# OpenSim2Real/gym-os2r

Hardware: AMD Instinct MI355X
Metric: env-steps/sec (aggregate) monopod balance task (higher is better)
Workload: dtype f64; 1 GPU; C4: 65536 envs/GPU free_hip balancing, ground contact, per-env domain randomisation (C5 = 8 x C4); envs_per_gpu=65536, total_envs=65536, task_mode=free_hip, substeps=10, pgs_exact=12, preroll_steps=1000, contact=True, domain_randomisation=True, actions=U(-1,1) Philox on device, n_ranks_seen=1, splits=1, rollout_steps_per_launch=1

## Files before the change

gym-os2r_amd/csrc/os2r_capi.hip:

```cpp
#include <hip/hip_runtime.h>

#include <cfloat>
#include <cmath>
#include <cstdio>
#include <cstring>
#include <new>
#include <deque>
#include <mutex>
#include <string>
#include <vector>

#include "os2r_kernels.hpp"

using namespace os2r;

namespace os2r {
int static_model_id(const Os2rModel& m);
bool same_model(const Os2rModel& a, const Os2rModel& b);
}

struct JitEntry {
  Os2rModel model;
  int dtype = 0, device = 0;
  hipModule_t module = nullptr;
// ... 61 lines not shown
  int32_t* steps = nullptr;
  uint32_t* episode = nullptr;
  uint8_t* pose = nullptr;
  void* solver_l = nullptr;
  uint32_t* solver_flags = nullptr;
  unsigned int* violations = nullptr;
  void *b_obs = nullptr, *b_rew = nullptr, *b_term = nullptr;
  unsigned long long* counters = nullptr;
  uint8_t* b_done = nullptr;
  hipEvent_t ev0 = nullptr, ev1 = nullptr;
  uint16_t* reason = nullptr;
  uint8_t* done_mask = nullptr;
  uint32_t* mirror_host = nullptr;
  uint32_t* mirror_dev = nullptr;
  unsigned long long* debug = nullptr;
  void* pol_act = nullptr;
  uint8_t* pol_open = nullptr;
  void* copy_stage = nullptr;
};

}

struct Os2rSim : SimBase {};

namespace {

#define HIP_TRY(sim, expr)                                                                     \
  do {                                                                                         \
    hipError_t _e = (expr);                                                                    \
    if (_e != hipSuccess) {                                                                    \
      (sim)->err = std::string(#expr) + ": " + hipGetErrorString(_e);                          \
      return OS2R_ERR_HIP;                                                                     \
    }                                                                                          \
  } while (0)

template <typename T>
void fill_model(const Os2rModel& m_in, bool contact, DevModel<T>& d) {
  Os2rModel m = m_in;
  if (!contact) m.ncand = 0;
  std::memset(&d, 0, sizeof(d));
  d.nq = m.nq;
  for (int i = 0; i < OS2R_MAX_DOF; ++i) {
    d.axis[i] = m.axis[i];
    for (int k = 0; k < 9; ++k) d.rfix[i][k] = (T)m.rfix[i][k];
    for (int k = 0; k < 3; ++k) { d.rpos[i][k] = (T)m.rpos[i][k]; d.com[i][k] = (T)m.com[i][k]; }
    for (int k = 0; k < 6; ++k) d.icom[i][k] = (T)m.icom[i][k];
    d.mass[i] = (T)m.mass[i];
    d.damping[i] = (T)m.damping[i];
    d.friction[i] = (T)m.friction[i];
    d.mu[i] = (T)m.mu[i];
  }
  for (int k = 0; k < 2; ++k) { d.act_dof[k] = m.act_dof[k]; d.max_torque[k] = (T)m.max_torque[k]; }
  d.gravity_z = (T)m.gravity_z;
  int k = 0;
  for (int b = 0; b < OS2R_MAX_DOF; ++b) {
    d.cand_begin[b] = k;
    while (k < m.ncand && m.cand_body[k] == b) ++k;
  }
  d.cand_begin[OS2R_MAX_DOF] = k;
  for (int c = 0; c < m.ncand; ++c)
    for (int j = 0; j < 3; ++j) d.cand_p[c][j] = (T)m.cand_p[c][j];
  for (int b = 0; b < OS2R_MAX_DOF; ++b) {
    for (int j = 0; j < 3; ++j) d.cand_center[b][j] = (T)m.cand_center[b][j];
    d.cand_radius[b] = m.cand_radius[b] > 0.0 ? (T)(m.cand_radius[b] * 1.000001) : (T)1e30;
  }
}

inline float float_at_or_above(double v) {
  float f = (float)v;
  if ((double)f < v) f = std::nextafter(f, FLT_MAX);
  return f;
}
inline float float_at_or_below(double v) {
  float f = (float)v;
  if ((double)f > v) f = std::nextafter(f, -FLT_MAX);
  return f;
}
inline void done_bounds(int kind, double lo, double hi, double& dlo, double& dhi) { dlo = lo; dhi = hi; }
inline void done_bounds(int kind, double lo, double hi, float& dlo, float& dhi) {
  const bool periodic = kind == OS2R_OBS_POS_PERIODIC_NORM || kind == OS2R_OBS_POS_PERIODIC_RAW;
  dlo = periodic ? float_at_or_below(lo) : float_at_or_above(lo);
  dhi = periodic ? float_at_or_above(hi) : float_at_or_below(hi);
}

template <typename T>
void fill_task(const Os2rConfig& cfg, DevTask<T>& d) {
  const Os2rTaskSpec& t = cfg.task;
  std::memset(&d, 0, sizeof(d));
  d.obs_dim = t.obs_dim;
  for (int i = 0; i < OS2R_MAX_OBS; ++i) {
    d.obs_kind[i] = t.obs_kind[i];
    d.obs_src[i] = t.obs_src[i];
    d.obs_low[i] = (T)t.obs_low[i];
    d.obs_high[i] = (T)t.obs_high[i];
    done_bounds(t.obs_kind[i], t.done_lo[i], t.done_hi[i], d.done_lo[i], d.done_hi[i]);
  }
  d.reward_id = t.reward_id; d.normalized = t.normalized;
  d.idx_pitch_pos = t.idx_pitch_pos; d.idx_yaw_vel = t.idx_yaw_vel;
  d.idx_hip_pos = t.idx_hip_pos; d.idx_knee_pos = t.idx_knee_pos;
  d.max_episode_steps = t.max_episode_steps;
  d.reset_mode = t.reset_mode; d.n_reset_poses = t.n_reset_poses;
  for (int i = 0; i < OS2R_MAX_RESET_POSES; ++i) {
    d.reset_pose_id[i] = t.reset_pose_id[i]; d.reset_laying[i] = t.reset_laying[i];
    d.reset_pitch[i] = t.reset_pitch[i]; d.reset_hip[i] = t.reset_hip[i]; d.reset_knee[i] = t.reset_knee[i];
  }
  d.reset_simple = t.reset_simple;
  for (int i = 0; i < 6; ++i) d.leg_def[i] = t.leg_def[i];
  d.dof_yaw = t.dof_yaw; d.dof_pitch = t.dof_pitch; d.dof_bc = t.dof_bc; d.dof_hip = t.dof_hip; d.dof_knee = t.dof_knee;
  d.randomize_params = t.randomize_params;
  d.gravity_rollouts = t.gravity_rollouts;
  d.dr_gravity_mean = t.dr_gravity_mean; d.dr_gravity_std = t.dr_gravity_std;
  d.dr_mass_lo = t.dr_mass_lo; d.dr_mass_hi = t.dr_mass_hi;
  d.dr_friction_lo = t.dr_friction_lo; d.dr_friction_hi = t.dr_friction_hi;
  d.dr_damping_lo = t.dr_damping_lo; d.dr_damping_hi = t.dr_damping_hi;
// ... 784 lines not shown
```

gym-os2r_amd/csrc/os2r_device.hpp:

```cpp
#pragma once
#include <type_traits>
#include <hip/hip_runtime.h>
#include <stdint.h>

#include "../../include/os2r.h"
#include "os2r_models_gen.hpp"

namespace os2r {

constexpr int kWave = 64;
template <typename T> struct StdSolver { static constexpr int kNormalIters = 2; static constexpr bool kExact = true; };
template <> struct StdSolver<float> { static constexpr int kNormalIters = 2; static constexpr bool kExact = false; };
__host__ __device__ constexpr int warm_first(int) { return 3; }
__host__ __device__ constexpr int sweep_cap_base(int nq) { return nq >= 5 ? 6 : 4; }
constexpr int kExactRounds = 8;
constexpr unsigned kCarryJoints = 0x80000000u;
template <typename T, int NQ_> struct SolverCarry {
  unsigned act = 0u;
  T ln[NQ_] = {}, lx[NQ_] = {}, ly[NQ_] = {}, lf[NQ_] = {};
};
template <typename T> __host__ __device__ constexpr int std_iters(int nq) { return sizeof(T) == 8 ? sweep_cap_base(nq) + kExactRounds : 20; }
template <typename T> __host__ __device__ inline bool is_std_solver(int iters, int normal_iters, int exact, int nq) {
  return iters == std_iters<T>(nq) && normal_iters == StdSolver<T>::kNormalIters && (exact > 0) == StdSolver<T>::kExact;
}
constexpr int kPgsGroup = 4;
constexpr int kExactProx = 2;
constexpr double kExactEps = 1e-6, kExactSnap = 1e-12;
constexpr double kExactIncons = 1e-4, kExactNoBound = 1e300;

struct WorkCounts {
  unsigned scanned = 0;
  unsigned row_bodies = 0;
  unsigned body_sweeps = 0;
  unsigned sweeps = 0;
  unsigned lane_contacts = 0;
  unsigned live_lane_sweeps = 0;
  unsigned full_sincos = 0;
  unsigned exact_solves = 0;
  unsigned lane_exact_solves = 0;
};

template <typename T>
struct DevModel {
  int nq;
  int axis[OS2R_MAX_DOF];
  T rfix[OS2R_MAX_DOF][9];
  T rpos[OS2R_MAX_DOF][3];
  T mass[OS2R_MAX_DOF];
  T com[OS2R_MAX_DOF][3];
  T icom[OS2R_MAX_DOF][6];
  T damping[OS2R_MAX_DOF];
  T friction[OS2R_MAX_DOF];
  T mu[OS2R_MAX_DOF];
  int act_dof[2];
  T max_torque[2];
  T gravity_z;
  int cand_begin[OS2R_MAX_DOF + 1];
  T cand_p[OS2R_MAX_CAND][3];
  T cand_center[OS2R_MAX_DOF][3];
  T cand_radius[OS2R_MAX_DOF];
};

template <typename T>
struct DevTask {
  int obs_dim;
  int obs_kind[OS2R_MAX_OBS];
  int obs_src[OS2R_MAX_OBS];
  T obs_low[OS2R_MAX_OBS];
  T obs_high[OS2R_MAX_OBS];
  T done_lo[OS2R_MAX_OBS];
  T done_hi[OS2R_MAX_OBS];
  int reward_id, normalized;
  int idx_pitch_pos, idx_yaw_vel, idx_hip_pos, idx_knee_pos;
  int max_episode_steps;
  int reset_mode, n_reset_poses;
  int reset_pose_id[OS2R_MAX_RESET_POSES];
  int reset_laying[OS2R_MAX_RESET_POSES];
  double reset_pitch[OS2R_MAX_RESET_POSES];
  double reset_hip[OS2R_MAX_RESET_POSES];
  double reset_knee[OS2R_MAX_RESET_POSES];
  int reset_simple;
  double leg_def[6];
  int dof_yaw, dof_pitch, dof_bc, dof_hip, dof_knee;
  int randomize_params;
  int gravity_rollouts;
  double dr_gravity_mean, dr_gravity_std;
  double dr_mass_lo, dr_mass_hi, dr_friction_lo, dr_friction_hi, dr_damping_lo, dr_damping_hi;
  double dr_mu_base, dr_mu_lo, dr_mu_hi;
  double nominal_damping[OS2R_MAX_DOF];
};

#define OS2R_CONST __attribute__((address_space(4)))
template <typename T> using ModelPtr = const OS2R_CONST DevModel<T>*;
template <typename T> using TaskPtr = const OS2R_CONST DevTask<T>*;
template <typename T> __device__ __forceinline__ ModelPtr<T> as_const(const DevModel<T>* p) { return (ModelPtr<T>)p; }
template <typename T> __device__ __forceinline__ TaskPtr<T> as_const(const DevTask<T>* p) { return (TaskPtr<T>)p; }

template <typename T>
struct StepArgs {
  const DevModel<T>* __restrict__ model;
  const DevTask<T>* __restrict__ task;
  long long N;
  long long env_offset;
  unsigned long long seed;
  unsigned long long step_count;
  int substeps;
  int rollout_steps;
  int pgs_iters;
  int pgs_normal_iters;
  int pgs_exact;
  int auto_reset;
  T dt, erp, max_erv, margin, gravity_z;
  T pgs_tol;
// ... 2 lines not shown
  T* __restrict__ hist;
  T* __restrict__ mass_scale;
  T* __restrict__ damping;
  T* __restrict__ friction;
  T* __restrict__ mu;
  T* __restrict__ gravity;
  int32_t* __restrict__ steps;
  uint32_t* __restrict__ episode;
  uint8_t* __restrict__ pose;
  T* __restrict__ solver_l;
  uint32_t* __restrict__ solver_flags;
  unsigned int* __restrict__ violations;
  const T* __restrict__ actions;
  T* __restrict__ obs;
  T* __restrict__ reward;
  uint8_t* __restrict__ done;
  T* __restrict__ term_obs;
  const uint8_t* __restrict__ reset_mask;
  unsigned long long* __restrict__ debug;
  unsigned long long* __restrict__ counters;
  uint16_t* __restrict__ reason;
  uint8_t* __restrict__ done_mask;
  uint32_t* __restrict__ mirror;
  unsigned long long layout_kinds, layout_srcs;
  int layout_dim;
};

template <typename T, int NQ_>
struct RtModel {
  static constexpr int NQ = NQ_;
  static constexpr unsigned CMASK = (1u << NQ_) - 1u;
  static constexpr bool kStatic = false;
  ModelPtr<T> p;
  __device__ __forceinline__ int axis(int i) const { return p->axis[i]; }
  __device__ __forceinline__ T rfix(int i, int k) const { return p->rfix[i][k]; }
  __device__ __forceinline__ T rpos(int i, int k) const { return p->rpos[i][k]; }
  __device__ __forceinline__ T mass(int i) const { return p->mass[i]; }
  __device__ __forceinline__ T com(int i, int k) const { return p->com[i][k]; }
  __device__ __forceinline__ T icom(int i, int k) const { return p->icom[i][k]; }
  __device__ __forceinline__ T damping(int i) const { return p->damping[i]; }
  __device__ __forceinline__ T friction(int i) const { return p->friction[i]; }
  __device__ __forceinline__ T mu(int i) const { return p->mu[i]; }
  __device__ __forceinline__ int act_dof(int k) const { return p->act_dof[k]; }
  __device__ __forceinline__ T max_torque(int k) const { return p->max_torque[k]; }
  __device__ __forceinline__ int cand_begin(int b) const { return p->cand_begin[b]; }
  __device__ __forceinline__ T cand(int k, int j) const { return p->cand_p[k][j]; }
  __device__ __forceinline__ T cand_center(int b, int j) const { return p->cand_center[b][j]; }
  __device__ __forceinline__ T cand_radius(int b) const { return p->cand_radius[b]; }
};

template <int ID>
struct CandMeta {
  using Tb = gen::Tables<ID>;
  struct Data { int axis[OS2R_MAX_DOF]; bool starts[OS2R_MAX_CAND > 0 ? OS2R_MAX_CAND : 1]; };
  static constexpr int runs(int b, int a) {
    int n = 0;
    for (int k = Tb::cand_begin[b]; k < Tb::cand_begin[b + 1]; ++k)
      if (k == Tb::cand_begin[b] || Tb::cand_p[k][a] != Tb::cand_p[k - 1][a]) ++n;
    return n;
  }
  static constexpr Data make() {
    Data d{};
    for (int b = 0; b < Tb::nq; ++b) {
      int best = 0;
      for (int a = 1; a < 3; ++a)
        if (runs(b, a) < runs(b, best)) best = a;
      d.axis[b] = best;
      for (int k = Tb::cand_begin[b]; k < Tb::cand_begin[b + 1]; ++k)
        d.starts[k] = k == Tb::cand_begin[b] || Tb::cand_p[k][best] != Tb::cand_p[k - 1][best];
    }
    return d;
  }
  static constexpr Data value = make();
};

template <typename T, int ID>
struct StModel {
  using Tb = gen::Tables<ID>;
  static constexpr int NQ = Tb::nq;
  static constexpr unsigned CMASK = Tb::cmask;
  static constexpr bool kStatic = true;
  __device__ __forceinline__ constexpr int axis(int i) const { return Tb::axis[i]; }
  __device__ __forceinline__ constexpr T rfix(int i, int k) const { return (T)Tb::rfix[i][k]; }
  __device__ __forceinline__ constexpr T rpos(int i, int k) const { return (T)Tb::rpos[i][k]; }
  __device__ __forceinline__ constexpr T mass(int i) const { return (T)Tb::mass[i]; }
  __device__ __forceinline__ constexpr T com(int i, int k) const { return (T)Tb::com[i][k]; }
  __device__ __forceinline__ constexpr T icom(int i, int k) const { return (T)Tb::icom[i][k]; }
  __device__ __forceinline__ constexpr T damping(int i) const { return (T)Tb::damping[i]; }
  __device__ __forceinline__ constexpr T friction(int i) const { return (T)Tb::friction[i]; }
  __device__ __forceinline__ constexpr T mu(int i) const { return (T)Tb::mu[i]; }
  __device__ __forceinline__ constexpr int act_dof(int k) const { return Tb::act_dof[k]; }
  __device__ __forceinline__ constexpr T max_torque(int k) const { return (T)Tb::max_torque[k]; }
  __device__ __forceinline__ constexpr int cand_begin(int b) const { return Tb::cand_begin[b]; }
  __device__ __forceinline__ constexpr T cand(int k, int j) const { return (T)Tb::cand_p[k][j]; }
  __device__ __forceinline__ constexpr T cand_center(int b, int j) const { return (T)Tb::cand_center[b][j]; }
  __device__ __forceinline__ constexpr T cand_radius(int b) const { return (T)Tb::cand_radius[b]; }
  static constexpr int cand_group_axis(int b) { return CandMeta<ID>::value.axis[b]; }
  static constexpr bool cand_starts_run(int , int k, int ) { return CandMeta<ID>::value.starts[k]; }
};

enum { kStreamAction = 1, kStreamReset = 2, kStreamParams = 3, kStreamGravity = 4, kStreamPolicyNoise = 5 };

__device__ __forceinline__ void philox4x32_10(uint32_t c0, uint32_t c1, uint32_t c2, uint32_t c3,
                                               uint32_t k0, uint32_t k1, uint32_t (&out)[4]) {
#pragma unroll
  for (int r = 0; r < 10; ++r) {
    const uint32_t hi0 = __umulhi(0xD2511F53u, c0), lo0 = 0xD2511F53u * c0;
    const uint32_t hi1 = __umulhi(0xCD9E8D57u, c2), lo1 = 0xCD9E8D57u * c2;
    const uint32_t n0 = hi1 ^ c1 ^ k0, n2 = hi0 ^ c3 ^ k1;
    c0 = n0; c1 = lo1; c2 = n2; c3 = lo0;
    k0 += 0x9E3779B9u; k1 += 0xBB67AE85u;
  }
  out[0] = c0; out[1] = c1; out[2] = c2; out[3] = c3;
}

__device__ __forceinline__ double u53(uint32_t a, uint32_t b) {
  return ((double)(a >> 5) * 67108864.0 + (double)(b >> 6)) / 9007199254740992.0;
}

__device__ __forceinline__ void uniform2(unsigned long long seed, uint32_t env, uint32_t stream,
                                          uint32_t ctr, uint32_t blk, double& u0, double& u1) {
  uint32_t o[4];
  philox4x32_10(env, stream, ctr, blk, (uint32_t)(seed & 0xffffffffull), (uint32_t)(seed >> 32), o);
  u0 = u53(o[0], o[1]);
  u1 = u53(o[2], o[3]);
}

__device__ __forceinline__ void normal2(unsigned long long seed, uint32_t env, uint32_t stream,
                                         uint32_t ctr, uint32_t blk, double& z0, double& z1) {
  double u0, u1;
  uniform2(seed, env, stream, ctr, blk, u0, u1);
  const double r = sqrt(-2.0 * log(1.0 - u0));
  const double th = 6.283185307179586476925286766559 * u1;
  z0 = r * cos(th);
  z1 = r * sin(th);
}

template <typename T>
struct V3 {
  T x, y, z;
};
template <typename T> __device__ __forceinline__ V3<T> mk(T x, T y, T z) { return V3<T>{x, y, z}; }
template <typename T> __device__ __forceinline__ V3<T> operator+(V3<T> a, V3<T> b) { return {a.x + b.x, a.y + b.y, a.z + b.z}; }
template <typename T> __device__ __forceinline__ V3<T> operator-(V3<T> a, V3<T> b) { return {a.x - b.x, a.y - b.y, a.z - b.z}; }
template <typename T> __device__ __forceinline__ V3<T> operator*(T s, V3<T> a) { return {s * a.x, s * a.y, s * a.z}; }
template <typename T> __device__ __forceinline__ T dot(V3<T> a, V3<T> b) { return a.x * b.x + a.y * b.y + a.z * b.z; }
template <typename T> __device__ __forceinline__ V3<T> cross(V3<T> a, V3<T> b) {
  return {a.y * b.z - a.z * b.y, a.z * b.x - a.x * b.z, a.x * b.y - a.y * b.x};
}
template <typename T> __device__ __forceinline__ T comp(V3<T> a, int k) { return k == 0 ? a.x : (k == 1 ? a.y : a.z); }
template <typename T> __device__ __forceinline__ void add_comp(V3<T>& a, int k, T v) {
// ... 153 lines not shown
  __device__ __forceinline__ T damping(int i) const { return slots[(1 * NQ + i) * kWave]; }
  __device__ __forceinline__ T friction(int i) const { return slots[(2 * NQ + i) * kWave]; }
  __device__ __forceinline__ T mu(int i) const { return slots[(3 * NQ + i) * kWave]; }
  __device__ __forceinline__ T gravity() const { return g; }
};

constexpr int kStamps = 32;
#if defined(OS2R_STAMPS) && defined(OS2R_STAMPS_LIGHT)
#define OS2R_STAMP(idx) do { } while (0)
#elif defined(OS2R_STAMPS)
#define OS2R_STAMP(idx)                                                                        \
  do {                                                                                         \
    __builtin_amdgcn_sched_barrier(0);                                                         \
    unsigned long long t_;                                                                     \
    asm volatile("s_memtime %0\n\ts_waitcnt lgkmcnt(0)" : "=s"(t_)::"memory");                 \
    __builtin_amdgcn_sched_barrier(0);                                                         \
    stamps[idx] += t_ - stamp_prev;                                                            \
    stamp_prev = t_;                                                                           \
  } while (0)
#elif defined(OS2R_PHASE_MARKS)
#define OS2R_STAMP(idx) asm volatile("s_nop 15\n\ts_nop %0\n\ts_nop %1" :: "i"((idx) % 8), "i"((idx) / 8) : "memory")
#else
#define OS2R_STAMP(idx) do { } while (0)
#endif

#ifdef OS2R_ISA_MARKS
#define OS2R_ISA_MARK(n) asm volatile("s_nop " #n ::: "memory")
#else
#define OS2R_ISA_MARK(n) do { } while (0)
#endif

constexpr int kPinVmem = 0x1 | 0x2 | 0x4 | 0x8 | 0x80 | 0x100 | 0x200 | 0x400;

constexpr int kPinDs = 0x1 | 0x2 | 0x4 | 0x8 | 0x10 | 0x20 | 0x40 | 0x400;

__device__ __forceinline__ double opaque(double x) { asm volatile("" : "+v"(x)); return x; }
__device__ __forceinline__ float opaque(float x) { asm volatile("" : "+v"(x)); return x; }

template <typename T> __device__ __forceinline__ T pick3(int k, T a, T b, T c) { return k == 0 ? a : (k == 1 ? b : c); }

template <typename T, typename MD>
__device__ __forceinline__ void joint_rotation(const MD& md, int i, T s_, T c_, T (&R)[9]) {
  const T s = opaque(s_), c = opaque(c_);
  const int ax = md.axis(i);
  const int ca = ax == 0 ? 1 : (ax == 1 ? 2 : 0);
  const int cb = ax == 0 ? 2 : (ax == 1 ? 0 : 1);
#pragma unroll
  for (int r = 0; r < 3; ++r) {
    const T fa = md.rfix(i, 3 * r + ca), fb = md.rfix(i, 3 * r + cb);
    const T keep = md.rfix(i, 3 * r + ax), va = c * fa + s * fb, vb = c * fb - s * fa;
#pragma unroll
    for (int j = 0; j < 3; ++j) R[3 * r + j] = j == ax ? keep : (j == ca ? va : vb);
  }
}

template <unsigned CMASK, int NB>
__device__ __forceinline__ constexpr int next_cand_body(int b) {
  for (int k = b + 1; k < NB; ++k)
    if ((CMASK >> k) & 1u) return k;
  return NB;
}
template <int B, int NB, unsigned CMASK, typename F>
__device__ __forceinline__ bool for_body(int b, F&& f) {
  if constexpr (B < NB) {
    if constexpr (((CMASK >> B) & 1u) && __builtin_popcount(CMASK >> B) <= 3) {
      if (b == B) { f(std::integral_constant<int, B>{}); return true; }
    }
    return for_body<B + 1, NB, CMASK>(b, f);
  } else {
    return false;
  }
}

enum { kSolverBoth = 0, kSolverExact = 1, kSolverSweeps = 2 };
template <typename T, typename MD, bool CONTACT, bool DR, bool COUNT = false, int SOLVER = kSolverBoth>
__device__ __forceinline__ void substep(const MD& md, const Params<T, MD, DR>& par,
                                        T (&q)[MD::NQ], T (&qd)[MD::NQ], T (&sn)[MD::NQ], T (&cs)[MD::NQ], bool first_iteration,
                                        T tau_hip, T tau_knee, T dt, T erp,
                                        T max_erv, T margin, int pgs_iters, int pgs_normal_iters, int pgs_exact, T pgs_tol, T* __restrict__ lds,
                                        const T* __restrict__ cand_lds, ModelPtr<T> mconst, WorkCounts& wc, SolverCarry<T, MD::NQ>& carry
#ifdef OS2R_STAMPS
                                        , unsigned long long (&stamps)[kStamps], unsigned long long& stamp_prev
#endif
                                        ) {
  constexpr int NQ = MD::NQ;
  constexpr unsigned CMASK = CONTACT ? MD::CMASK : 0u;
  const T inv_dt = rcp_t(dt);
  const T m_first = par.mass(NQ - 1), damp_first = par.damping(NQ - 1);
  __builtin_amdgcn_sched_barrier(DR ? kPinDs : kPinVmem);
  {
    bool ok = true, small = !first_iteration;
#pragma unroll
    for (int i = 0; i < NQ; ++i) { ok = ok && sincos_in_range(q[i]); small = small && fabs_t(dt * qd[i]) < T(0.06); }
    if constexpr (COUNT) wc.full_sincos += __ballot(!small) != 0ull ? 1u : 0u;
    if (small) {
#pragma unroll
      for (int i = 0; i < NQ; ++i) {
        const T d = dt * qd[i], z = d * d;
        T p = fma_t(z, T(-1.0 / 39916800.0), T(1.0 / 362880.0));
        p = fma_t(z, p, T(-1.0 / 5040.0));
        p = fma_t(z, p, T(1.0 / 120.0));
        p = fma_t(z, p, T(-1.0 / 6.0));
        const T sd = fma_t(d * z, p, d);
        T r = fma_t(z, T(-1.0 / 3628800.0), T(1.0 / 40320.0));
        r = fma_t(z, r, T(-1.0 / 720.0));
        r = fma_t(z, r, T(1.0 / 24.0));
// ... 234 lines not shown
#pragma unroll
      for (int r = i; r < NQ; ++r) Lc[r][i] = r == i ? sdi : uk[r][i] * sdi;
    }
  }
  OS2R_STAMP(19);

  OS2R_STAMP(2);
  T fb[NQ];
  T mub[NB];
#pragma unroll
  for (int j = 0; j < NQ; ++j) fb[j] = par.friction(j);
#pragma unroll
  for (int b = 0; b < NB; ++b) mub[b] = ((CMASK >> b) & 1u) ? par.mu(b) : T(0);
  __builtin_amdgcn_sched_barrier(DR ? kPinDs : kPinVmem);
  T y[NQ];
  T idj[NQ];
#pragma unroll
  for (int j = 0; j < NQ; ++j) {
    T mjj = 0;
#pragma unroll
    for (int k = 0; k <= j; ++k) { mjj += Lc[j][k] * Lc[j][k]; Lcs(j, k) = Lc[j][k]; }
    idj[j] = mjj > T(0) ? rcp_t(mjj) : T(0);
  }
#pragma unroll
  for (int i = 0; i < NQ; ++i) {
    T acc_ = vs[i];
#pragma unroll
    for (int k = 0; k < i; ++k) acc_ -= Lc[i][k] * y[k];
    y[i] = opaque(acc_ * Ldi[i]);
  }
  constexpr bool kStdExact = sizeof(T) == 8 && SOLVER == kSolverExact && MD::kStatic;
  constexpr bool kParkY0 = sizeof(T) == 8 && !kStdExact && (SOLVER != kSolverSweeps || !MD::kStatic);
  constexpr int kY0Slot = NQ * (NQ + 1) / 2 + 3 * NQ + NQ;
  static_assert(kY0Slot + NQ <= 8 * NQ, "per-lane LDS slots");
  T y0[NQ];
#pragma unroll
  for (int i = 0; i < NQ; ++i) {
    if constexpr (kParkY0) L(kY0Slot + i) = y[i];
    else y0[i] = y[i];
  }

  OS2R_STAMP(3);
  T dn[NB], dx[NB], dy[NB], erv[NB];
  T Gr[NB][3][NQ];
  bool act[NB];
  bool wave_act[NB];
#pragma unroll
  for (int b = 0; b < NB; ++b) { act[b] = false; wave_act[b] = false; }
  if (CMASK != 0u) {
    T Rw[9], ow[3];
    V3<T> aw[NQ], jo[NQ];
#pragma unroll
    for (int b = 0; b < NB; ++b) {
      constexpr int CHS = 4;
      T bA[3 * CHS], bB[3 * CHS];
      auto request = [&](int kk, int kend, T (&d)[3 * CHS]) {
#pragma unroll
        for (int j = 0; j < 3 * CHS; ++j) d[j] = (kk + j / 3 < kend) ? mconst->cand_p[kk + j / 3][j % 3] : T(0);
      };
      if constexpr (MD::kStatic) {
        if ((CMASK >> b) & 1u) {
          request(md.cand_begin(b), md.cand_begin(b + 1), bA);
          asm volatile("" ::: "memory");
        }
      }
      const V3<T> r = mk(md.rpos(b, 0), md.rpos(b, 1), md.rpos(b, 2));
      T Rb[9];
      joint_rotation<T>(md, b, sn[b], cs[b], Rb);
      if (b == 0) {
#pragma unroll
        for (int k = 0; k < 9; ++k) Rw[k] = Rb[k];
        ow[0] = r.x; ow[1] = r.y; ow[2] = r.z;
      } else {
        const V3<T> t = rmul(Rw, r);
        ow[0] += t.x; ow[1] += t.y; ow[2] += t.z;
        T n[9];
#pragma unroll
        for (int i = 0; i < 3; ++i)
#pragma unroll
          for (int j = 0; j < 3; ++j) n[3 * i + j] = Rw[3 * i] * Rb[j] + Rw[3 * i + 1] * Rb[3 + j] + Rw[3 * i + 2] * Rb[6 + j];
#pragma unroll
        for (int k = 0; k < 9; ++k) Rw[k] = n[k];
      }
      const int ax = md.axis(b);
      aw[b] = mk(pick3(ax, Rw[0], Rw[1], Rw[2]), pick3(ax, Rw[3], Rw[4], Rw[5]), pick3(ax, Rw[6], Rw[7], Rw[8]));
      jo[b] = mk(ow[0], ow[1], ow[2]);
      if (!((CMASK >> b) & 1u)) continue;
      OS2R_STAMP(4);
      const int k0 = md.cand_begin(b), k1 = md.cand_begin(b + 1);
      T W = 0, sx = 0, sy = 0, sz = 0;
      const T zc = Rw[6] * md.cand_center(b, 0) + Rw[7] * md.cand_center(b, 1) + Rw[8] * md.cand_center(b, 2) + ow[2];
      const bool near = zc - md.cand_radius(b) < margin;
      if constexpr (MD::kStatic) {
#pragma unroll
        for (int j = 0; j < 3 * CHS; ++j) asm volatile("" : "+s"(bA[j]));
        asm volatile("" ::: "memory");
      }
      if constexpr (COUNT) wc.scanned += __ballot(near) != 0ull ? 1u : 0u;
      if (__ballot(near) != 0ull)
      {
        constexpr int CH = 4;
        auto fetch = [&](int k, T (&d)[3 * CH]) {
#pragma unroll
          for (int j = 0; j < 3 * CH; ++j) d[j] = cand_lds[3 * k + j];
        };
        auto consume = [&](const T (&d)[3 * CH]) {
#pragma unroll
          for (int c = 0; c < CH; ++c) {
            const T px = d[3 * c], py = d[3 * c + 1], pz = d[3 * c + 2];
            const T z = Rw[6] * px + Rw[7] * py + Rw[8] * pz + ow[2];
            const T wgt = fmax_t(margin - z, T(0));
            W += wgt; sx += wgt * px; sy += wgt * py; sz += wgt * pz;
          }
        };
        if constexpr (MD::kStatic) {
          const T mo = margin - ow[2];
          auto arrived = [&](T (&d)[3 * CH]) {
#pragma unroll
            for (int j = 0; j < 3 * CH; ++j) asm volatile("" : "+s"(d[j]));
            asm volatile("" ::: "memory");
          };
          const int ga = MD::cand_group_axis(b), a1 = (ga + 1) % 3, a2 = (ga + 2) % 3;
          T S[3] = {T(0), T(0), T(0)};
          T Wg = T(0), pg = T(0), base = mo;
          auto weigh = [&](const T (&d)[3 * CH], int kk) {
#pragma unroll
            for (int c = 0; c < CH; ++c) {
              if (kk + c < k1) {
                if (MD::cand_starts_run(b, kk + c, ga)) {
                  W += Wg; S[ga] = fma_t(pg, Wg, S[ga]);
                  Wg = T(0); pg = d[3 * c + ga];
                  base = fma_t(-Rw[6 + ga], pg, mo);
                }
                const T p1 = d[3 * c + a1], p2 = d[3 * c + a2];
                const T mz = fma_t(-Rw[6 + a1], p1, fma_t(-Rw[6 + a2], p2, base));
                const T wgt = fmax_t(mz, T(0));
                Wg += wgt; S[a1] = fma_t(wgt, p1, S[a1]); S[a2] = fma_t(wgt, p2, S[a2]);
              }
            }
          };
          static_assert(CH == CHS, "chunk size of the request issued ahead");
#pragma unroll
          for (int kk = k0; kk < k1; kk += 2 * CH) {
            arrived(bA);
            if (kk + CH < k1) request(kk + CH, k1, bB);
            weigh(bA, kk);
            if (kk + CH < k1) {
              arrived(bB);
              if (kk + 2 * CH < k1) request(kk + 2 * CH, k1, bA);
              weigh(bB, kk + CH);
            }
          }
          W += Wg; S[ga] = fma_t(pg, Wg, S[ga]);
          sx = S[0]; sy = S[1]; sz = S[2];
        } else {
        T bufA[3 * CH], bufB[3 * CH];
        int k = k0;
        const int kpair = k0 + ((k1 - k0) / (2 * CH)) * (2 * CH);
        if (k < kpair) {
          fetch(k, bufA);
#pragma unroll 1
          for (; k < kpair; k += 2 * CH) {
            fetch(k + CH, bufB);
            consume(bufA);
            if (k + 2 * CH < kpair) fetch(k + 2 * CH, bufA);
            consume(bufB);
          }
        }
#pragma unroll 1
        for (; k < k1; ++k) {
          const T px = cand_lds[3 * k], py = cand_lds[3 * k + 1], pz = cand_lds[3 * k + 2];
          const T z = Rw[6] * px + Rw[7] * py + Rw[8] * pz + ow[2];
          const T wgt = fmax_t(margin - z, T(0));
          W += wgt; sx += wgt * px; sy += wgt * py; sz += wgt * pz;
        }
        }
      }
      OS2R_STAMP(5);
      act[b] = W > T(0);
      wave_act[b] = __ballot(act[b]) != 0ull;
      if constexpr (COUNT) { wc.row_bodies += wave_act[b] ? 1u : 0u; wc.lane_contacts += (unsigned)__popcll(__ballot(act[b])); }
      if (wave_act[b]) {
        T lcb[NQ][NQ];
#pragma unroll
        for (int j = 0; j < NQ; ++j)
#pragma unroll
          for (int k = 0; k < NQ; ++k)
            if (j <= b && k <= j) lcb[j][k] = Lcs(j, k);
        __builtin_amdgcn_sched_barrier(kPinDs);
        const T iw = act[b] ? rcp_t(W) : T(0);
        const V3<T> pc = mk(sx * iw, sy * iw, sz * iw);
        const V3<T> pw = rmul(Rw, pc) + jo[b];
        const T gap = pw.z;
        const T e = erp * (-gap) * inv_dt;
        erv[b] = gap >= T(0) ? -gap * inv_dt : (e > max_erv ? max_erv : e);
        T Jn[NQ], Jx[NQ], Jy[NQ];
#pragma unroll
        for (int j = 0; j < NQ; ++j) {
          if (j <= b) {
            const V3<T> c = cross(aw[j], pw - jo[j]);
            Jx[j] = c.x; Jy[j] = c.y; Jn[j] = c.z;
          }
        }
// ... 492 lines not shown
```

gym-os2r_amd/csrc/os2r_pybind.cpp:

```cpp
#include <pybind11/pybind11.h>
#include <pybind11/stl.h>

#include <cstdint>

#include "../../include/os2r.h"

namespace py = pybind11;
using addr = std::uintptr_t;

static Os2rSim* H(addr h) { return reinterpret_cast<Os2rSim*>(h); }
static void* P(addr a) { return reinterpret_cast<void*>(a); }

PYBIND11_MODULE(_os2r_py, m) {
  m.doc() = "pybind11 binding of libos2r.so (MI355X batched monopod stepper)";
  const auto nogil = py::call_guard<py::gil_scoped_release>();
  m.def("abi_version", &os2r_abi_version);
  m.def("abi_minor", &os2r_abi_minor);
  m.def("create", [](addr cfg) {
    Os2rSim* s = nullptr;
    int rc;
    { py::gil_scoped_release rel; rc = os2r_create(reinterpret_cast<const Os2rConfig*>(cfg), &s); }
    return py::make_tuple(rc, reinterpret_cast<addr>(s));
  });
  m.def("destroy", [](addr h) { return os2r_destroy(H(h)); }, nogil);
  m.def("reset", [](addr h, addr mask, addr obs, addr st) { return os2r_reset(H(h), (const uint8_t*)P(mask), P(obs), P(st)); }, nogil);
  m.def("step", [](addr h, addr act, addr obs, addr rew, addr done, addr term, addr st) {
    return os2r_step(H(h), P(act), P(obs), P(rew), (uint8_t*)P(done), P(term), P(st)); }, nogil);
  m.def("rollout", [](addr h, int n, addr act, addr obs, addr rew, addr done, addr term, addr why, addr st) {
    return os2r_rollout(H(h), n, P(act), P(obs), P(rew), (uint8_t*)P(done), P(term), (uint16_t*)P(why), P(st)); }, nogil);
  m.def("rollout_policy", [](addr h, int n, addr w, int flags, addr ret, addr len, addr obs, addr rew, addr done, addr term, addr why,
                             addr st) {
    return os2r_rollout_policy(H(h), n, P(w), flags, P(ret), (int32_t*)P(len), P(obs), P(rew), (uint8_t*)P(done), P(term),
                               (uint16_t*)P(why), P(st)); }, nogil);
  m.def("rollout_policy_noisy", [](addr h, int n, addr w, int flags, addr sigma, uint32_t salt, addr ret, addr len, addr obs, addr rew,
                                   addr done, addr term, addr why, addr act, addr eps, addr st) {
    return os2r_rollout_policy_noisy(H(h), n, P(w), flags, P(sigma), salt, P(ret), (int32_t*)P(len), P(obs), P(rew), (uint8_t*)P(done),
                                     P(term), (uint16_t*)P(why), P(act), P(eps), P(st)); }, nogil);
  m.def("rollout_policy_scheduled", [](addr h, int n, addr w, int period, int first, int flags, addr sigma, uint32_t salt, addr ret,
                                       addr len, addr obs, addr rew, addr done, addr term, addr why, addr act, addr eps, addr st) {
    return os2r_rollout_policy_scheduled(H(h), n, P(w), period, first, flags, P(sigma), salt, P(ret), (int32_t*)P(len), P(obs), P(rew),
                                         (uint8_t*)P(done), P(term), (uint16_t*)P(why), P(act), P(eps), P(st)); }, nogil);
  m.def("copy_envs", [](addr dst, addr src, addr index, int what, addr obs, addr st) {
    return os2r_copy_envs(H(dst), H(src), (const int32_t*)P(index), what, P(obs), P(st)); }, nogil);
  m.def("linearize", [](addr h, addr act, double eq, double ev, double ea, addr next, addr ja, addr jb, addr st) {
    const double eps[3] = {eq, ev, ea};
    return os2r_linearize(H(h), P(act), eps, P(next), P(ja), P(jb), P(st)); }, nogil);
  m.def("get_solver_state", [](addr h, addr l, addr f, addr st) { return os2r_get_solver_state(H(h), P(l), (uint32_t*)P(f), P(st)); }, nogil);
  m.def("set_solver_state", [](addr h, addr l, addr f, addr st) { return os2r_set_solver_state(H(h), P(l), (const uint32_t*)P(f), P(st)); }, nogil);
  m.def("get_state", [](addr h, addr q, addr qd, addr st) { return os2r_get_state(H(h), P(q), P(qd), P(st)); }, nogil);
  m.def("set_state", [](addr h, addr q, addr qd, addr st) { return os2r_set_state(H(h), P(q), P(qd), P(st)); }, nogil);
  m.def("get_action_history", [](addr h, int w, addr o, addr st) { return os2r_get_action_history(H(h), w, P(o), P(st)); }, nogil);
  m.def("set_action_history", [](addr h, int w, addr i, addr st) { return os2r_set_action_history(H(h), w, P(i), P(st)); }, nogil);
  m.def("set_params", [](addr h, int f, addr s, addr st) { return os2r_set_params(H(h), f, P(s), P(st)); }, nogil);
  m.def("get_params", [](addr h, int f, addr d, addr st) { return os2r_get_params(H(h), f, P(d), P(st)); }, nogil);
  m.def("get_episode_info", [](addr h, addr s, addr e, addr p, addr st) {
    return os2r_get_episode_info(H(h), (int32_t*)P(s), (uint32_t*)P(e), (uint8_t*)P(p), P(st)); }, nogil);
  m.def("set_episode_info", [](addr h, addr s, addr e, addr p, addr st) {
    return os2r_set_episode_info(H(h), (const int32_t*)P(s), (const uint32_t*)P(e), (const uint8_t*)P(p), P(st)); }, nogil);
  m.def("get_action_violations", [](addr h, addr d, int clear, addr st) {
    return os2r_get_action_violations(H(h), (uint32_t*)P(d), clear, P(st)); }, nogil);
  m.def("get_step_count", [](addr h) { uint64_t v = 0; int rc = os2r_get_step_count(H(h), &v); return py::make_tuple(rc, v); });
  m.def("set_step_count", [](addr h, uint64_t v) { return os2r_set_step_count(H(h), v); });
  m.def("bench_steps", [](addr h, int n, addr st) {
    float ms = 0.f;
    int rc;
    { py::gil_scoped_release rel; rc = os2r_bench_steps(H(h), n, P(st), &ms); }
    return py::make_tuple(rc, ms);
  });
  m.def("bench_enqueue", [](addr h, int n, addr st) {
    py::gil_scoped_release rel;
    return os2r_bench_steps(H(h), n, P(st), nullptr);
  });
  m.def("bench_steps_multi", [](std::vector<addr> hs, std::vector<addr> sts, int n) {
    std::vector<Os2rSim*> sims; std::vector<void*> streams;
    for (addr h : hs) sims.push_back(H(h));
    for (addr s : sts) streams.push_back(P(s));
    if (sims.size() != streams.size()) return (int)OS2R_ERR_INVALID;
    py::gil_scoped_release rel;
    return os2r_bench_steps_multi(sims.data(), streams.data(), (int)sims.size(), n);
  });
  m.def("set_work_counters", [](addr h, addr buf) { return os2r_set_work_counters(H(h), (uint64_t*)P(buf)); });
  m.def("set_done_reasons", [](addr h, addr buf) { return os2r_set_done_reasons(H(h), (uint16_t*)P(buf)); });
  m.def("set_done_mask", [](addr h, addr buf) { return os2r_set_done_mask(H(h), (uint8_t*)P(buf)); });
  m.def("get_violation_mirror", [](addr h) { const volatile uint32_t* w = nullptr; int rc = os2r_get_violation_mirror(H(h), &w); return py::make_tuple(rc, (addr)w); });
  m.def("model_is_compiled_in", [](addr model) { return os2r_model_is_compiled_in((const Os2rModel*)P(model)); });
  m.def("register_model_kernels", [](addr model, int dtype, int device, const std::string& path) {
    return os2r_register_model_kernels((const Os2rModel*)P(model), dtype, device, path.c_str()); });
  m.def("last_error", [](addr h) { return std::string(os2r_last_error(H(h))); });
}
```

gym-os2r_amd/jit.py:

```python
from __future__ import annotations

import ctypes as C
import hashlib
import os
import shutil
import subprocess
import tempfile
import warnings

from . import abi

_HERE = os.path.dirname(os.path.abspath(__file__))
CSRC = os.path.join(_HERE, "csrc")
ARCH = "gfx950"
FLAGS = ["-O3", "-std=c++17", "-fno-signed-zeros", "-fno-honor-nans", "-fno-honor-infinities", "-fno-slp-vectorize",
         "-mllvm", "-disable-machine-licm", "-mllvm", "-disable-machine-sink"]
_registered = set()


def enabled() -> bool:
    return os.environ.get("OS2R_JIT", "1") not in ("0", "false", "off", "")


def hipcc_path():
# ... 11 lines not shown

def _hx(x) -> str:
    return float(x).hex()


def table_source(m: abi.Os2rModel, table_id: int = 100) -> str:
    nq, nc = int(m.nq), int(m.ncand)
    begins, k = [], 0
    for b in range(nq):
        begins.append(k)
        while k < nc and m.cand_body[k] == b:
            k += 1
    begins.append(k)
    if k != nc:
        raise ValueError("candidate points must be grouped by body in ascending order")
    cmask = 0
    for c in range(nc):
        cmask |= 1 << int(m.cand_body[c])

    def arr1(vals):
        return "{" + ", ".join(vals) + "}"

    def arr2(rows):
        return "{" + ", ".join(arr1([_hx(v) for v in r]) for r in rows) + "}"

    cand = [[m.cand_p[c][j] for j in range(3)] for c in range(nc)] or [[0.0, 0.0, 0.0]]
    out = ["// GENERATED by gym_os2r_amd/jit.py -- the constants of one robot, numbers only.", "#pragma once",
           "namespace os2r { namespace gen {", f"template <> struct Tables<{table_id}> {{",
           f"  static constexpr int nq = {nq};",
           f"  static constexpr unsigned cmask = {cmask}u;",
           f"  static constexpr int axis[{nq}] = {arr1([str(int(m.axis[i])) for i in range(nq)])};",
           f"  static constexpr double rfix[{nq}][9] = {arr2([[m.rfix[i][k] for k in range(9)] for i in range(nq)])};",
           f"  static constexpr double rpos[{nq}][3] = {arr2([[m.rpos[i][k] for k in range(3)] for i in range(nq)])};",
           f"  static constexpr double mass[{nq}] = {arr1([_hx(m.mass[i]) for i in range(nq)])};",
           f"  static constexpr double com[{nq}][3] = {arr2([[m.com[i][k] for k in range(3)] for i in range(nq)])};",
           f"  static constexpr double icom[{nq}][6] = {arr2([[m.icom[i][k] for k in range(6)] for i in range(nq)])};",
           f"  static constexpr double damping[{nq}] = {arr1([_hx(m.damping[i]) for i in range(nq)])};",
           f"  static constexpr double friction[{nq}] = {arr1([_hx(m.friction[i]) for i in range(nq)])};",
           f"  static constexpr double mu[{nq}] = {arr1([_hx(m.mu[i]) for i in range(nq)])};",
           f"  static constexpr int act_dof[2] = {{{int(m.act_dof[0])}, {int(m.act_dof[1])}}};",
           f"  static constexpr double max_torque[2] = {{{_hx(m.max_torque[0])}, {_hx(m.max_torque[1])}}};",
           f"  static constexpr int ncand = {nc};",
           f"  static constexpr int cand_begin[{nq + 1}] = {arr1([str(v) for v in begins])};",
           f"  static constexpr double cand_p[{max(nc, 1)}][3] = {arr2(cand)};",
           f"  static constexpr double cand_center[{nq}][3] = "
           f"{arr2([[m.cand_center[i][k] for k in range(3)] for i in range(nq)])};",
           f"  static constexpr double cand_radius[{nq}] = {arr1([_hx(m.cand_radius[i]) for i in range(nq)])};",
           "};", "} }  // namespace os2r::gen", ""]
    return "\n".join(out)


def _sources_digest() -> str:
    h = hashlib.sha256()
    for name in ("os2r_device.hpp", "os2r_kernels.hpp", "os2r_models_gen.hpp", "os2r_jit_unit.hip"):
        with open(os.path.join(CSRC, name), "rb") as f:
            h.update(f.read())
    with open(os.path.join(os.path.dirname(_HERE), "include", "os2r.h"), "rb") as f:
        h.update(f.read())
    return h.hexdigest()


def task_layout(task: abi.Os2rTaskSpec):
    dim = int(task.obs_dim)
    if not 0 < dim <= abi.MAX_OBS or any(not 0 <= int(task.obs_kind[d]) < 16 or not 0 <= int(task.obs_src[d]) < 16 for d in range(dim)):
        return None
    kinds = sum(int(task.obs_kind[d]) << (4 * d) for d in range(dim))
    srcs = sum(int(task.obs_src[d]) << (4 * d) for d in range(dim))
    return kinds, srcs, dim


def code_object_path(m: abi.Os2rModel, dtype: int, contact: bool, layout=None) -> str:
    h = hashlib.sha256()
    h.update(table_source(m).encode())
    h.update(f"{dtype}|{int(bool(contact))}|{layout if contact else None}|{ARCH}|{' '.join(FLAGS)}|{_sources_digest()}".encode())
    return os.path.join(cache_dir(), f"os2r_{h.hexdigest()[:24]}.hsaco")


def build(m: abi.Os2rModel, dtype: int, contact: bool, force: bool = False, layout=None) -> str:
    out = code_object_path(m, dtype, contact, layout)
    if os.path.exists(out) and not force:
        return out
    hipcc = hipcc_path()
    if hipcc is None:
        raise RuntimeError("hipcc not found (set HIPCC or install ROCm): cannot specialise the kernels")
    real = "double" if dtype == abi.F64 else "float"
    with tempfile.TemporaryDirectory(prefix="os2r_jit_") as tmp:
        tab = os.path.join(tmp, "os2r_jit_tables.hpp")
        with open(tab, "w") as f:
            f.write(table_source(m))
        obj = os.path.join(tmp, "unit.hsaco")
        cmd = [hipcc, "--genco", f"--offload-arch={ARCH}", *FLAGS, f"-DOS2R_REAL={real}",
               f"-DOS2R_JIT_CONTACT={int(bool(contact))}", f'-DOS2R_JIT_TABLES="{tab}"', f"-I{CSRC}",
               *([f"-DOS2R_JIT_LAYOUT_KINDS={layout[0]}ull", f"-DOS2R_JIT_LAYOUT_SRCS={layout[1]}ull",
                  f"-DOS2R_JIT_LAYOUT_DIM={layout[2]}"] if (layout and contact) else []),
               os.path.join(CSRC, "os2r_jit_unit.hip"), "-o", obj]
        r = subprocess.run(cmd, stdout=subprocess.PIPE, stderr=subprocess.STDOUT, text=True)
        if r.returncode != 0 or not os.path.exists(obj):
            raise RuntimeError("hipcc failed on the specialised kernels:\n" + r.stdout[-4000:])
        tmp_out = f"{out}.{os.getpid()}.tmp"
        shutil.copyfile(obj, tmp_out)
        os.replace(tmp_out, out)
    return out


def specialise(lib, cfg: abi.Os2rConfig) -> bool:
    if not enabled():
        return False
# ... 15 lines not shown
```

Measured before the change: 495.0 million env-steps/s.

## Pack contact candidates into two-axis pairs and load with wide vector loads

Adds a packed copy of each contact candidate that keeps only the two non-group axes, and takes the group-axis value from compile-time metadata. The static contact scan now reads 2 values per candidate instead of 3, using wide vector loads into scalar registers, and the chunk size rises from 4 to 6. The aim is to cut constant-memory loads and scalar register pressure in the ground-contact candidate scan. In exchange the device model struct grows, and the larger chunk may raise SGPR use.

After: 498.4 million env-steps/s (median of 6 runs). No clear change (+0.7%).

```diff
diff --git a/gym-os2r_amd/csrc/os2r_cand_pack.hpp b/gym-os2r_amd/csrc/os2r_cand_pack.hpp
--- /dev/null
+++ b/gym-os2r_amd/csrc/os2r_cand_pack.hpp
@@ -0,0 +1,55 @@
+#pragma once
+
+#if defined(__HIPCC__) || defined(__CUDACC__)
+#define OS2R_HD __host__ __device__
+#else
+#define OS2R_HD
+#endif
+
+namespace os2r {
+
+
+template <class P>
+OS2R_HD constexpr int cand_runs(const P& p, int k0, int k1, int a) {
+  int n = 0;
+  for (int k = k0; k < k1; ++k)
+    if (k == k0 || p[k][a] != p[k - 1][a]) ++n;
+  return n;
+}
+
+template <class P>
+OS2R_HD constexpr int cand_group_axis_of(const P& p, int k0, int k1) {
+  int best = 0;
+  for (int a = 1; a < 3; ++a)
+    if (cand_runs(p, k0, k1, a) < cand_runs(p, k0, k1, best)) best = a;
+  return best;
+}
+
+template <class P>
+OS2R_HD constexpr bool cand_run_start(const P& p, int k0, int k, int a) {
+  return k == k0 || p[k][a] != p[k - 1][a];
+}
+
+OS2R_HD constexpr int cand_packed_axis(int group_axis, int slot) { return (group_axis + 1 + slot) % 3; }
+
+template <class B>
+inline void cand_begins(const B& body, int ncand, int nbody, int* begin) {
+  int k = 0;
+  for (int b = 0; b < nbody; ++b) {
+    begin[b] = k;
+    while (k < ncand && body[k] == b) ++k;
+  }
+  begin[nbody] = k;
+}
+
+template <class T, class P, class Q>
+inline void cand_pack(const P& p, const int* begin, int nbody, Q& pk, int* axis_out) {
+  for (int b = 0; b < nbody; ++b) {
+    const int ga = cand_group_axis_of(p, begin[b], begin[b + 1]);
+    if (axis_out) axis_out[b] = ga;
+    for (int k = begin[b]; k < begin[b + 1]; ++k)
+      for (int s = 0; s < 2; ++s) pk[k][s] = (T)p[k][cand_packed_axis(ga, s)];
+  }
+}
+
+}
diff --git a/gym-os2r_amd/csrc/os2r_capi.hip b/gym-os2r_amd/csrc/os2r_capi.hip
--- a/gym-os2r_amd/csrc/os2r_capi.hip
+++ b/gym-os2r_amd/csrc/os2r_capi.hip
@@ -137,14 +137,10 @@
   }
   for (int k = 0; k < 2; ++k) { d.act_dof[k] = m.act_dof[k]; d.max_torque[k] = (T)m.max_torque[k]; }
   d.gravity_z = (T)m.gravity_z;
-  int k = 0;
-  for (int b = 0; b < OS2R_MAX_DOF; ++b) {
-    d.cand_begin[b] = k;
-    while (k < m.ncand && m.cand_body[k] == b) ++k;
-  }
-  d.cand_begin[OS2R_MAX_DOF] = k;
+  cand_begins(m.cand_body, m.ncand, OS2R_MAX_DOF, d.cand_begin);
   for (int c = 0; c < m.ncand; ++c)
     for (int j = 0; j < 3; ++j) d.cand_p[c][j] = (T)m.cand_p[c][j];
+  cand_pack<T>(m.cand_p, d.cand_begin, OS2R_MAX_DOF, d.cand_pk, nullptr);
   for (int b = 0; b < OS2R_MAX_DOF; ++b) {
     for (int j = 0; j < 3; ++j) d.cand_center[b][j] = (T)m.cand_center[b][j];
     d.cand_radius[b] = m.cand_radius[b] > 0.0 ? (T)(m.cand_radius[b] * 1.000001) : (T)1e30;
diff --git a/gym-os2r_amd/csrc/os2r_device.hpp b/gym-os2r_amd/csrc/os2r_device.hpp
--- a/gym-os2r_amd/csrc/os2r_device.hpp
+++ b/gym-os2r_amd/csrc/os2r_device.hpp
@@ -5,10 +5,14 @@
 
 #include "../../include/os2r.h"
 #include "os2r_models_gen.hpp"
+#include "os2r_cand_pack.hpp"
 
 namespace os2r {
 
 constexpr int kWave = 64;
+#ifndef OS2R_SCAN_CHUNK
+#define OS2R_SCAN_CHUNK 6
+#endif
 template <typename T> struct StdSolver { static constexpr int kNormalIters = 2; static constexpr bool kExact = true; };
 template <> struct StdSolver<float> { static constexpr int kNormalIters = 2; static constexpr bool kExact = false; };
 __host__ __device__ constexpr int warm_first(int) { return 3; }
@@ -59,6 +63,7 @@
   T cand_p[OS2R_MAX_CAND][3];
   T cand_center[OS2R_MAX_DOF][3];
   T cand_radius[OS2R_MAX_DOF];
+  T cand_pk[OS2R_MAX_CAND][2];
 };
 
 template <typename T>
@@ -167,22 +172,17 @@
 template <int ID>
 struct CandMeta {
   using Tb = gen::Tables<ID>;
-  struct Data { int axis[OS2R_MAX_DOF]; bool starts[OS2R_MAX_CAND > 0 ? OS2R_MAX_CAND : 1]; };
-  static constexpr int runs(int b, int a) {
-    int n = 0;
-    for (int k = Tb::cand_begin[b]; k < Tb::cand_begin[b + 1]; ++k)
-      if (k == Tb::cand_begin[b] || Tb::cand_p[k][a] != Tb::cand_p[k - 1][a]) ++n;
-    return n;
-  }
+  struct Data { int axis[OS2R_MAX_DOF]; bool starts[OS2R_MAX_CAND > 0 ? OS2R_MAX_CAND : 1]; double group[OS2R_MAX_CAND > 0 ? OS2R_MAX_CAND : 1]; };
   static constexpr Data make() {
     Data d{};
     for (int b = 0; b < Tb::nq; ++b) {
-      int best = 0;
-      for (int a = 1; a < 3; ++a)
-        if (runs(b, a) < runs(b, best)) best = a;
+      const int k0 = Tb::cand_begin[b], k1 = Tb::cand_begin[b + 1];
+      const int best = cand_group_axis_of(Tb::cand_p, k0, k1);
       d.axis[b] = best;
-      for (int k = Tb::cand_begin[b]; k < Tb::cand_begin[b + 1]; ++k)
-        d.starts[k] = k == Tb::cand_begin[b] || Tb::cand_p[k][best] != Tb::cand_p[k - 1][best];
+      for (int k = k0; k < k1; ++k) {
+        d.starts[k] = cand_run_start(Tb::cand_p, k0, k, best);
+        d.group[k] = Tb::cand_p[k][best];
+      }
     }
     return d;
   }
@@ -212,6 +212,7 @@
   __device__ __forceinline__ constexpr T cand_radius(int b) const { return (T)Tb::cand_radius[b]; }
   static constexpr int cand_group_axis(int b) { return CandMeta<ID>::value.axis[b]; }
   static constexpr bool cand_starts_run(int , int k, int ) { return CandMeta<ID>::value.starts[k]; }
+  static constexpr T cand_group_value(int k) { return (T)CandMeta<ID>::value.group[k]; }
 };
 
 enum { kStreamAction = 1, kStreamReset = 2, kStreamParams = 3, kStreamGravity = 4, kStreamPolicyNoise = 5 };
@@ -471,6 +472,15 @@
 #pragma unroll
     for (int j = 0; j < 3; ++j) R[3 * r + j] = j == ax ? keep : (j == ca ? va : vb);
   }
+}
+
+template <int W, typename T>
+__device__ __forceinline__ void load_wide(const OS2R_CONST T* p, T* d) {
+  typedef T Vec __attribute__((ext_vector_type(W)));
+  typedef Vec VecU __attribute__((aligned(sizeof(T))));
+  const VecU v = *(const OS2R_CONST VecU*)p;
+#pragma unroll
+  for (int i = 0; i < W; ++i) d[i] = v[i];
 }
 
 template <unsigned CMASK, int NB>
@@ -811,11 +821,19 @@
     V3<T> aw[NQ], jo[NQ];
 #pragma unroll
     for (int b = 0; b < NB; ++b) {
-      constexpr int CHS = 4;
-      T bA[3 * CHS], bB[3 * CHS];
-      auto request = [&](int kk, int kend, T (&d)[3 * CHS]) {
-#pragma unroll
-        for (int j = 0; j < 3 * CHS; ++j) d[j] = (kk + j / 3 < kend) ? mconst->cand_p[kk + j / 3][j % 3] : T(0);
+      constexpr int CHS = OS2R_SCAN_CHUNK;
+      T bA[2 * CHS], bB[2 * CHS];
+      auto request = [&](int kk, int kend, T (&d)[2 * CHS]) {
+        const int n = 2 * (kend - kk < CHS ? kend - kk : CHS);
+        const OS2R_CONST T* p = &mconst->cand_pk[kk][0];
+#pragma unroll
+        for (int j = 0; j < 2 * CHS; ++j) d[j] = T(0);
+        int o = 0;
+#pragma unroll
+        for (int r = 0; r < (2 * CHS) / 8; ++r)
+          if (n - o >= 8) { load_wide<8>(p + o, d + o); o += 8; }
+        if (n - o >= 4) { load_wide<4>(p + o, d + o); o += 4; }
+        if (n - o >= 2) { load_wide<2>(p + o, d + o); o += 2; }
       };
       if constexpr (MD::kStatic) {
         if ((CMASK >> b) & 1u) {
@@ -852,7 +870,7 @@
       const bool near = zc - md.cand_radius(b) < margin;
       if constexpr (MD::kStatic) {
 #pragma unroll
-        for (int j = 0; j < 3 * CHS; ++j) asm volatile("" : "+s"(bA[j]));
+        for (int j = 0; j < 2 * CHS; ++j) asm volatile("" : "+s"(bA[j]));
         asm volatile("" ::: "memory");
       }
       if constexpr (COUNT) wc.scanned += __ballot(near) != 0ull ? 1u : 0u;
@@ -874,40 +892,41 @@
         };
         if constexpr (MD::kStatic) {
           const T mo = margin - ow[2];
-          auto arrived = [&](T (&d)[3 * CH]) {
-#pragma unroll
-            for (int j = 0; j < 3 * CH; ++j) asm volatile("" : "+s"(d[j]));
+          constexpr int CP = CHS;
+          auto arrived = [&](T (&d)[2 * CP]) {
+#pragma unroll
+            for (int j = 0; j < 2 * CP; ++j) asm volatile("" : "+s"(d[j]));
             asm volatile("" ::: "memory");
           };
           const int ga = MD::cand_group_axis(b), a1 = (ga + 1) % 3, a2 = (ga + 2) % 3;
           T S[3] = {T(0), T(0), T(0)};
           T Wg = T(0), pg = T(0), base = mo;
-          auto weigh = [&](const T (&d)[3 * CH], int kk) {
-#pragma unroll
-            for (int c = 0; c < CH; ++c) {
+          static_assert(cand_packed_axis(0, 0) == 1 && cand_packed_axis(0, 1) == 2 && cand_packed_axis(2, 0) == 0, "order of the packed pair");
+          auto weigh = [&](const T (&d)[2 * CP], int kk) {
+#pragma unroll
+            for (int c = 0; c < CP; ++c) {
               if (kk + c < k1) {
                 if (MD::cand_starts_run(b, kk + c, ga)) {
                   W += Wg; S[ga] = fma_t(pg, Wg, S[ga]);
-                  Wg = T(0); pg = d[3 * c + ga];
+                  Wg = T(0); pg = MD::cand_group_value(kk + c);
                   base = fma_t(-Rw[6 + ga], pg, mo);
                 }
-                const T p1 = d[3 * c + a1], p2 = d[3 * c + a2];
+                const T p1 = d[2 * c], p2 = d[2 * c + 1];
                 const T mz = fma_t(-Rw[6 + a1], p1, fma_t(-Rw[6 + a2], p2, base));
                 const T wgt = fmax_t(mz, T(0));
                 Wg += wgt; S[a1] = fma_t(wgt, p1, S[a1]); S[a2] = fma_t(wgt, p2, S[a2]);
               }
             }
           };
-          static_assert(CH == CHS, "chunk size of the request issued ahead");
-#pragma unroll
-          for (int kk = k0; kk < k1; kk += 2 * CH) {
+#pragma unroll
+          for (int kk = k0; kk < k1; kk += 2 * CP) {
             arrived(bA);
-            if (kk + CH < k1) request(kk + CH, k1, bB);
+            if (kk + CP < k1) request(kk + CP, k1, bB);
             weigh(bA, kk);
-            if (kk + CH < k1) {
+            if (kk + CP < k1) {
               arrived(bB);
-              if (kk + 2 * CH < k1) request(kk + 2 * CH, k1, bA);
-              weigh(bB, kk + CH);
+              if (kk + 2 * CP < k1) request(kk + 2 * CP, k1, bA);
+              weigh(bB, kk + CP);
             }
           }
           W += Wg; S[ga] = fma_t(pg, Wg, S[ga]);
diff --git a/gym-os2r_amd/csrc/os2r_pybind.cpp b/gym-os2r_amd/csrc/os2r_pybind.cpp
--- a/gym-os2r_amd/csrc/os2r_pybind.cpp
+++ b/gym-os2r_amd/csrc/os2r_pybind.cpp
@@ -4,6 +4,7 @@
 #include <cstdint>
 
 #include "../../include/os2r.h"
+#include "os2r_cand_pack.hpp"
 
 namespace py = pybind11;
 using addr = std::uintptr_t;
@@ -84,6 +85,24 @@
   m.def("set_done_mask", [](addr h, addr buf) { return os2r_set_done_mask(H(h), (uint8_t*)P(buf)); });
   m.def("get_violation_mirror", [](addr h) { const volatile uint32_t* w = nullptr; int rc = os2r_get_violation_mirror(H(h), &w); return py::make_tuple(rc, (addr)w); });
   m.def("model_is_compiled_in", [](addr model) { return os2r_model_is_compiled_in((const Os2rModel*)P(model)); });
+  m.def("pack_candidates", [](addr model) {
+    const Os2rModel& mo = *(const Os2rModel*)P(model);
+    int begin[OS2R_MAX_DOF + 1], axis[OS2R_MAX_DOF];
+    double pk[OS2R_MAX_CAND][2] = {};
+    os2r::cand_begins(mo.cand_body, mo.ncand, OS2R_MAX_DOF, begin);
+    os2r::cand_pack<double>(mo.cand_p, begin, OS2R_MAX_DOF, pk, axis);
+    py::list b, a, p, s, g;
+    for (int i = 0; i <= OS2R_MAX_DOF; ++i) b.append(begin[i]);
+    for (int i = 0; i < OS2R_MAX_DOF; ++i) {
+      a.append(axis[i]);
+      for (int k = begin[i]; k < begin[i + 1]; ++k) {
+        p.append(py::make_tuple(pk[k][0], pk[k][1]));
+        s.append(os2r::cand_run_start(mo.cand_p, begin[i], k, axis[i]));
+        g.append(mo.cand_p[k][axis[i]]);
+      }
+    }
+    return py::make_tuple(b, a, p, s, g);
+  });
   m.def("register_model_kernels", [](addr model, int dtype, int device, const std::string& path) {
     return os2r_register_model_kernels((const Os2rModel*)P(model), dtype, device, path.c_str()); });
   m.def("last_error", [](addr h) { return std::string(os2r_last_error(H(h))); });
diff --git a/gym-os2r_amd/jit.py b/gym-os2r_amd/jit.py
--- a/gym-os2r_amd/jit.py
+++ b/gym-os2r_amd/jit.py
@@ -87,7 +87,7 @@
 
 def _sources_digest() -> str:
     h = hashlib.sha256()
-    for name in ("os2r_device.hpp", "os2r_kernels.hpp", "os2r_models_gen.hpp", "os2r_jit_unit.hip"):
+    for name in ("os2r_device.hpp", "os2r_kernels.hpp", "os2r_models_gen.hpp", "os2r_cand_pack.hpp", "os2r_jit_unit.hip"):
         with open(os.path.join(CSRC, name), "rb") as f:
             h.update(f.read())
     with open(os.path.join(os.path.dirname(_HERE), "include", "os2r.h"), "rb") as f:
```
